# AE-HYU/monte_carlo_localization

Hardware: AMD Instinct MI355X
Metric: MCL updates/sec (particle*beam/s) (higher is better)
Workload: dtype f64; 1 GPU; 4194304 particles/GPU x 1081 beams, Spielberg_map (2000x2000 @ 0.05796), initial cloud N((0.0, 0.0, 0.0),(0.5 m,0.5 m,0.4 rad)) (tracking regime), action (0.05, 0.0, 0.01), stock sensor/motion params, multinomial resampling, Philox seed 42; the timed updates follow 5 warm-up updates (the particle set has resampled to motion-noise width); particles_total=4194304, beams=1081, parallelism=single GPU

## Files before the change

monte_carlo_localization_amd/csrc/mcl_kernels.h:

```cpp
#pragma once
#include "mcl_types.h"
#include <type_traits>
#include "mcl_ray_core.h"
#include "mcl_device_math.h"
#include "mcl_wedge.h"
#include "mcl_motion.h"

namespace mcl {

constexpr int kRedBlocks = 1024;
constexpr int kRedThreads = 256;
__device__ __forceinline__ void final_sums_of(const double *__restrict__ part, int nb, double *__restrict__ scalars, double (*sm)[7]);


__device__ __forceinline__ uint64_t wave_incl_scan_u64(uint64_t v, int lane)
{
#pragma unroll
    for (int o = 1; o < 64; o <<= 1) {
        uint64_t t = (uint64_t)__shfl_up((long long)v, o, 64);
        if (lane >= o) v += t;
    }
    return v;
}

// ... 1204 lines not shown
__global__ __launch_bounds__(1024) void k_tile_compact(int *__restrict__ bbox, int *__restrict__ tilemark, int *__restrict__ tilemap, int ntiles_abs)
{
    __shared__ int ws[16];
    __shared__ int carry_sh;
    const int lane = threadIdx.x & 63, wv = threadIdx.x >> 6;
    if (threadIdx.x == 0) carry_sh = 0;
    __syncthreads();
    for (int t0 = 0; t0 < ntiles_abs; t0 += 1024) {
        const int t = t0 + (int)threadIdx.x;
        const int m = (t < ntiles_abs && tilemark[t] != 0) ? 1 : 0;
        int inc = m;
#pragma unroll
        for (int o = 1; o < 64; o <<= 1) { const int v = __shfl_up(inc, o, 64); if (lane >= o) inc += v; }
        if (lane == 63) ws[wv] = inc;
        __syncthreads();
        int id = carry_sh + inc - m;
        for (int k = 0; k < wv; ++k) id += ws[k];
        if (t < ntiles_abs) { tilemap[t] = m ? id : -1; tilemark[t] = 0; }
        __syncthreads();
        if (threadIdx.x == 1023) carry_sh = id + m;
        __syncthreads();
    }
    const int T = carry_sh;
    for (int t = threadIdx.x; t < ntiles_abs; t += 1024)
        if (tilemap[t] < 0) tilemap[t] = T;
    if (threadIdx.x == 0) { bbox[4] = T; bbox[5] = 1; }
}

#ifndef MCL_SORT_SUB_GATE
#define MCL_SORT_SUB_GATE 32.0
#endif
constexpr double kSortSubGate = MCL_SORT_SUB_GATE;
constexpr int kSortMaxSub = MCL_SORT_MAX_SUB;
struct SortLayout {
    int cs, tb, inner, ss;
    uint32_t ntx;
    int tx0, ty0;
    bool compact;
    bool nocut;
    bool sparse;
    uint64_t ntiles;
    __device__ __forceinline__ int tile_shift() const { return 2 * inner + 2 * ss + tb; }
    __device__ __forceinline__ int cut_shift() const { return sparse ? 2 * ss + tb : tile_shift(); }
    __device__ __forceinline__ uint64_t cut_groups() const { return sparse ? ntiles << (2 * inner) : ntiles; }
    __device__ __forceinline__ bool cuts() const;
};
constexpr int kSwMaxCuts = 65536;
__device__ __forceinline__ bool SortLayout::cuts() const
{
    return compact && !nocut && cut_groups() <= (uint64_t)kSwMaxCuts && (cut_groups() << cut_shift()) <= kSortKeySpace;
}
__device__ __forceinline__ SortLayout sort_layout(const int *__restrict__ bbox, int64_t n)
{
    SortLayout L;
    L.tx0 = bbox[0] >> 5; L.ty0 = bbox[1] >> 5;
    L.ntx = (uint32_t)((bbox[2] >> 5) - L.tx0 + 1);
    const uint32_t nty = (uint32_t)((bbox[3] >> 5) - L.ty0 + 1);
    L.compact = bbox[5] != 0;
    L.ntiles = L.compact ? (uint64_t)bbox[4] + 1u : (uint64_t)L.ntx * nty;
    double cells_est = (double)(bbox[2] - bbox[0] + 1) * (double)(bbox[3] - bbox[1] + 1);
    if (L.compact && (double)bbox[4] * 1024.0 < cells_est) cells_est = (double)bbox[4] * 1024.0;
    int cs = 0, tb = 6;
    L.nocut = bbox[6] < 0;
    L.sparse = cells_est > 0.0 && (double)n < 8.0 * cells_est;
    if (L.sparse) {
        cs = 5;
        const int play = bbox[6];
        while (play > 0 && cs > 1 && (1 << cs) >= play - 2 && (double)n * (double)(1 << (2 * cs - 2)) >= 128.0 * cells_est) --cs;
    }
    while (cs < 5 && ((L.ntiles << (10 - 2 * cs + tb)) > kSortKeySpace)) ++cs;
    while (tb > 0 && ((L.ntiles << (10 - 2 * cs + tb)) > kSortKeySpace)) --tb;
    const int inner = 5 - cs;
    const uint64_t ncell = L.ntiles << (2 * inner);
    while (tb < 8 && (ncell << (tb + 1)) <= kSortKeySpace) ++tb;
    int ss = 0;
    if (cs == 0 && tb == 8) {
        double per_bucket = cells_est > 0.0 ? (double)n / cells_est / 32.0 : 0.0;
        while (ss < kSortMaxSub && (ncell << (tb + 2 * (ss + 1))) <= kSortKeySpace && per_bucket >= kSortSubGate) { ++ss; per_bucket *= 0.25; }
    }
    L.cs = cs; L.tb = tb; L.inner = inner; L.ss = ss;
    return L;
}

__device__ __forceinline__ uint32_t sort_key(const int *__restrict__ bbox, const int *__restrict__ tilemap, int ntx_abs, int cx, int cy, double th,
                                         int64_t n, double fx, double fy)
{
    cx = cx < bbox[0] ? bbox[0] : (cx > bbox[2] ? bbox[2] : cx);
    cy = cy < bbox[1] ? bbox[1] : (cy > bbox[3] ? bbox[3] : cy);
    const SortLayout L = sort_layout(bbox, n);
    const int cs = L.cs, tb = L.tb, inner = L.inner, ss = L.ss;
    uint32_t tile = (uint32_t)((cy >> 5) - L.ty0) * L.ntx + (uint32_t)((cx >> 5) - L.tx0);
    if (L.compact) tile = (uint32_t)tilemap[(cy >> 5) * ntx_abs + (cx >> 5)];
    const uint32_t ix = (uint32_t)(cx & 31) >> cs, iy = (uint32_t)(cy & 31) >> cs;
    uint64_t key = ((((uint64_t)tile << inner) | iy) << inner) | ix;
    if (ss > 0) {
        const uint32_t sx = (fx >= 0.0 && fx < 1.0) ? (uint32_t)(fx * (double)(1 << ss)) : 0u;
        const uint32_t sy = (fy >= 0.0 && fy < 1.0) ? (uint32_t)(fy * (double)(1 << ss)) : 0u;
        key = (((key << ss) | sy) << ss) | sx;
    }
    double f = th * 0.15915494309189533577;
    f -= floor(f);
    uint32_t tq = (f >= 0.0 && f < 1.0) ? (uint32_t)(f * (double)(1u << tb)) : 0u;
    if (tq >> tb) tq = (1u << tb) - 1u;
    key = (key << tb) | tq;
    return key < kSortKeySpace ? (uint32_t)key : kSortKeySpace - 1u;
}

__global__ __launch_bounds__(256) void k_sort_hist(const double4 *__restrict__ pc, const double *__restrict__ th, int64_t n, int Wp, int Hp,
                                                  const int *__restrict__ bbox, uint32_t *__restrict__ hist,
                                                  uint32_t *__restrict__ key_out, uint32_t *__restrict__ rank_out, uint32_t *__restrict__ tile_used,
                                                  const int *__restrict__ tilemap, int ntx_abs)
{
    const int64_t i = (int64_t)blockIdx.x * blockDim.x + threadIdx.x;
    if (i >= n) return;
    const uint32_t xcd = (uint32_t)__builtin_amdgcn_s_getreg((20 << 0) | (0 << 6) | (3 << 11)) & (kSortXcds - 1);
    const double4 c = pc[i];
    const uint32_t key = sort_key(bbox, tilemap, ntx_abs, cell_of(c.z * kSortSub, Wp * kSortSub - 1), cell_of(c.w * kSortSub, Hp * kSortSub - 1), th[i], n,
                                  c.z * kSortSub - floor(c.z * kSortSub), c.w * kSortSub - floor(c.w * kSortSub));
    key_out[i] = key;
    const uint32_t r = __hip_atomic_fetch_add(&hist[(size_t)xcd * kSortKeySpace + key], 1u, __ATOMIC_RELAXED, __HIP_MEMORY_SCOPE_WORKGROUP);
    rank_out[i] = (xcd << 28) | r;
    if (r == 0u) tile_used[key / kHistTile] = 1u;
}

__global__ __launch_bounds__(256) void k_hist_partials(const uint32_t *__restrict__ hist, uint32_t *__restrict__ part, const uint32_t *__restrict__ tile_used)
{
    __shared__ uint32_t ws[4];
    if (!tile_used[blockIdx.x]) {
        if (threadIdx.x == 0) part[blockIdx.x] = 0u;
        return;
    }
    uint32_t s = 0;
    for (int x = 0; x < kSortXcds; ++x) {
        const uint4 *p = reinterpret_cast<const uint4 *>(hist + (size_t)x * kSortKeySpace + (size_t)blockIdx.x * kHistTile) + threadIdx.x * 4;
#pragma unroll
        for (int k = 0; k < 4; ++k) { uint4 v = p[k]; s += v.x + v.y + v.z + v.w; }
    }
#pragma unroll
    for (int o = 32; o > 0; o >>= 1) s += __shfl_xor(s, o, 64);
    if ((threadIdx.x & 63) == 0) ws[threadIdx.x >> 6] = s;
    __syncthreads();
    if (threadIdx.x == 0) part[blockIdx.x] = ws[0] + ws[1] + ws[2] + ws[3];
}

__global__ __launch_bounds__(256) void k_hist_final(uint32_t *__restrict__ hist, const uint32_t *__restrict__ part, const uint32_t *__restrict__ tile_used)
{
    __shared__ uint32_t ws[4], ps[4];
    if (!tile_used[blockIdx.x]) return;
    const int lane = threadIdx.x & 63, w = threadIdx.x >> 6;
    uint32_t pre = 0;
    for (int t = (int)threadIdx.x; t < (int)blockIdx.x; t += 256) pre += part[t];
#pragma unroll
    for (int o = 32; o > 0; o >>= 1) pre += __shfl_xor(pre, o, 64);
    if (lane == 0) ps[w] = pre;
    const size_t b0 = (size_t)blockIdx.x * kHistTile + (size_t)threadIdx.x * 16;
    uint4 v[kSortXcds][4];
    uint32_t s = 0;
#pragma unroll
    for (int x = 0; x < kSortXcds; ++x) {
        const uint4 *p = reinterpret_cast<const uint4 *>(hist + (size_t)x * kSortKeySpace + b0);
#pragma unroll
        for (int k = 0; k < 4; ++k) { v[x][k] = p[k]; s += v[x][k].x + v[x][k].y + v[x][k].z + v[x][k].w; }
    }
    uint32_t inc = s;
#pragma unroll
    for (int o = 1; o < 64; o <<= 1) { uint32_t t = __shfl_up(inc, o, 64); if (lane >= o) inc += t; }
    if (lane == 63) ws[w] = inc;
    __syncthreads();
    uint32_t run = ps[0] + ps[1] + ps[2] + ps[3] + inc - s;
    for (int k = 0; k < w; ++k) run += ws[k];
#pragma unroll
    for (int k = 0; k < 4; ++k) {
#pragma unroll
        for (int x = 0; x < kSortXcds; ++x) { uint32_t c = v[x][k].x; v[x][k].x = run; run += c; }
#pragma unroll
        for (int x = 0; x < kSortXcds; ++x) { uint32_t c = v[x][k].y; v[x][k].y = run; run += c; }
#pragma unroll
        for (int x = 0; x < kSortXcds; ++x) { uint32_t c = v[x][k].z; v[x][k].z = run; run += c; }
#pragma unroll
        for (int x = 0; x < kSortXcds; ++x) { uint32_t c = v[x][k].w; v[x][k].w = run; run += c; }
    }
#pragma unroll
    for (int x = 0; x < kSortXcds; ++x) {
        uint4 *p = reinterpret_cast<uint4 *>(hist + (size_t)x * kSortKeySpace + b0);
#pragma unroll
        for (int k = 0; k < 4; ++k) p[k] = v[x][k];
    }
}

__global__ __launch_bounds__(256) void k_sort_scatter(const double4 *__restrict__ pc, const double *__restrict__ th, int64_t n,
                                                     const uint32_t *__restrict__ key, const uint32_t *__restrict__ rank,
                                                     const uint32_t *__restrict__ start, double4 *__restrict__ pcs,
                                                     double *__restrict__ ths, uint32_t *__restrict__ perm)
{
    const int64_t i = (int64_t)blockIdx.x * blockDim.x + threadIdx.x;
    if (i >= n) return;
    const uint32_t rk = rank[i];
    const uint32_t slot = start[(size_t)(rk >> 28) * kSortKeySpace + key[i]] + (rk & 0x0FFFFFFFu);
    if (slot >= (uint64_t)n) return;
    pcs[slot] = pc[i];
    ths[slot] = th[i];
    perm[slot] = (uint32_t)i;
}

__global__ __launch_bounds__(256) void k_sort_keys(const double4 *__restrict__ pc, const double *__restrict__ th, int64_t n, int Wp, int Hp,
                                                  const int *__restrict__ bbox, uint32_t *__restrict__ key_out, uint32_t *__restrict__ val_out,
                                                  const int *__restrict__ tilemap, int ntx_abs)
{
    const int64_t i = (int64_t)blockIdx.x * blockDim.x + threadIdx.x;
    if (i >= n) return;
    const double4 c = pc[i];
    key_out[i] = sort_key(bbox, tilemap, ntx_abs, cell_of(c.z * kSortSub, Wp * kSortSub - 1), cell_of(c.w * kSortSub, Hp * kSortSub - 1), th[i], n,
                          c.z * kSortSub - floor(c.z * kSortSub), c.w * kSortSub - floor(c.w * kSortSub));
    val_out[i] = (uint32_t)i;
}
__global__ __launch_bounds__(256) void k_sort_gather(const double4 *__restrict__ pc, const double *__restrict__ th, int64_t n,
                                                    const uint32_t *__restrict__ order, double4 *__restrict__ pcs, double *__restrict__ ths,
                                                    uint32_t *__restrict__ perm, const uint32_t *__restrict__ sorted_keys = nullptr,
                                                    const int *__restrict__ bbox = nullptr, uint32_t *__restrict__ cut_start = nullptr,
                                                    uint32_t *__restrict__ cut_end = nullptr)
{
    const int64_t s = (int64_t)blockIdx.x * blockDim.x + threadIdx.x;
    if (s >= n) return;
    const uint32_t i = order[s];
    pcs[s] = pc[i];
    ths[s] = th[i];
    perm[s] = i;
    if (sorted_keys) {
        const SortLayout L = sort_layout(bbox, n);
        if (L.cuts()) {
            const int sh = L.cut_shift();
            const uint32_t g = sorted_keys[s] >> sh;
            const uint32_t gp = s > 0 ? sorted_keys[s - 1] >> sh : 0xFFFFFFFFu;
            if (g != gp && g < (uint32_t)kSwMaxCuts) {
                cut_start[g] = (uint32_t)s + 1u;
                if (s > 0 && gp < (uint32_t)kSwMaxCuts) cut_end[gp] = (uint32_t)s;
            }
            if (s == n - 1 && g < (uint32_t)kSwMaxCuts) cut_end[g] = (uint32_t)n;
        }
    }
}

__global__ __launch_bounds__(256) void k_hist_clear(uint32_t *__restrict__ hist, uint32_t *__restrict__ tile_used)
{
    if (!tile_used[blockIdx.x]) return;
    const uint4 z = make_uint4(0u, 0u, 0u, 0u);
    for (int x = 0; x < kSortXcds; ++x) {
        uint4 *p = reinterpret_cast<uint4 *>(hist + (size_t)x * kSortKeySpace + (size_t)blockIdx.x * kHistTile) + threadIdx.x * 4;
#pragma unroll
        for (int k = 0; k < 4; ++k) p[k] = z;
    }
    __syncthreads();
    if (threadIdx.x == 0) tile_used[blockIdx.x] = 0u;
}

__global__ __launch_bounds__(256) void k_slice_means(const double4 *__restrict__ pcs, int64_t n, int64_t per, double2 *__restrict__ out)
{
    __shared__ double sm[4][3];
    const int64_t p_begin = (int64_t)blockIdx.x * per;
    const int64_t p_end = (p_begin + per < n) ? p_begin + per : n;
    double sx = 0.0, sy = 0.0, cnt = 0.0;
    for (int64_t s = p_begin + threadIdx.x; s < p_end; s += blockDim.x) {
        const double4 c = pcs[s];
        if (c.z == c.z && c.w == c.w && fabs(c.z) < 1e9 && fabs(c.w) < 1e9) { sx += c.z; sy += c.w; cnt += 1.0; }
    }
    sx = wave_sum(sx); sy = wave_sum(sy); cnt = wave_sum(cnt);
    if ((threadIdx.x & 63) == 0) { sm[threadIdx.x >> 6][0] = sx; sm[threadIdx.x >> 6][1] = sy; sm[threadIdx.x >> 6][2] = cnt; }
    __syncthreads();
    if (threadIdx.x == 0) {
        sx = sm[0][0] + sm[1][0] + sm[2][0] + sm[3][0];
        sy = sm[0][1] + sm[1][1] + sm[2][1] + sm[3][1];
        cnt = sm[0][2] + sm[1][2] + sm[2][2] + sm[3][2];
        out[blockIdx.x] = cnt > 0.0 ? make_double2(sx / cnt, sy / cnt) : make_double2(0.0, 0.0);
    }
}

template <bool GRID = false>
__device__ __forceinline__ int first_beam_in_wedge(double th, const float *__restrict__ angle, int B, int m, double a0, double inv_inc)
{
    int lo = 0, hi = B;
    const double x = ((double)m * (6.283185307179586476925286766559 / kWedges) - th - a0) * inv_inc;
    if (x > -4.0 && x < (double)B + 4.0) {
        const int jg = min(max((int)ceil(x), 0), B);
        if (GRID && fabs(x - rint(x)) > 4e-6 * inv_inc + 1e-6) return jg;
        const bool below = jg == 0 || beam_wedge(th, angle[jg - 1]) < m;
        const bool at = jg == B || beam_wedge(th, angle[jg]) >= m;
        if (below && at) return jg;
        const int l = max(jg - 2, 0), h = min(jg + 2, B);
        if ((l == 0 || beam_wedge(th, angle[l - 1]) < m) && (h == B || beam_wedge(th, angle[h]) >= m)) { lo = l; hi = h; }
    }
    while (lo < hi) {
        const int mid = (lo + hi) >> 1;
        if (beam_wedge(th, angle[mid]) >= m) hi = mid; else lo = mid + 1;
    }
    return lo;
}

#ifdef MCL_LEGACY_RAY_KERNELS
}
#include "mcl_rays_legacy.h"
namespace mcl {
#endif

template <bool COUNT>
__global__ __launch_bounds__(256) void k_rays_fix(RayArgs a)
{
    unsigned long long cnt_exact = 0, cnt_probe = 0, cnt_l2 = 0;
    const int split = max(1, (int)gridDim.x / a.fix_segments);
    const int part = blockIdx.x % split;
    for (int seg = blockIdx.x / split; seg < a.fix_segments; seg += gridDim.x / split) {
    unsigned long long n = 0;
    if (threadIdx.x == 0) n = a.slot_space ? a.fix_count[(size_t)seg * 8] : atomicAdd(&a.fix_count[(size_t)seg * 8], 0ull);
    n = __shfl((long long)n, 0, 64);
    {
        __shared__ unsigned long long n_sh;
        if (threadIdx.x == 0) n_sh = n;
        __syncthreads();
        n = n_sh;
        __syncthreads();
    }
    if (n > a.fix_cap) n = 0;
    cnt_l2 += (threadIdx.x == 0 && part == 0) ? n : 0;
    const unsigned long long *list = a.fix_list + (size_t)seg * a.fix_cap;
    for (unsigned long long k = (unsigned long long)part * blockDim.x + threadIdx.x; k < n; k += (unsigned long long)blockDim.x * split) {
        const unsigned long long e = a.slot_space ? list[k] : atomicAdd(const_cast<unsigned long long *>(&list[k]), 0ull);
        const int64_t p = (int64_t)(e >> 16);
        const int j = (int)(e & 0xFFFF);
        const double4 pci = a.slot_space ? a.pcs[p] : a.pc[p];
        const uint8_t *wfield = nullptr;
        if (a.slot_space && a.distw) {
            const double hth = a.ths[p];
            if (hth == hth && fabs(hth) < 1e6) wfield = a.distw + (size_t)(beam_wedge(hth, a.beam_angle[j]) & (kWedges - 1)) * a.distw_stride;
        }
        const double2 cs = a.beam_cs[j];
        const double ux = pci.x * cs.x - pci.y * cs.y, uy = pci.y * cs.x + pci.x * cs.y;
        const RayOrigin o = ray_origin(a, pci.z, pci.w);
        int r = a.P;
        uint32_t amb = o.amb0;
        unsigned np = 0;
        if (o.sane)
            r = trace_fp64<false, COUNT>(a, nullptr, 0, kOriginBase, o.p0x, o.p0y, ux, uy, first_skip(a, o, wfield ? wfield : a.dist, wfield != nullptr),
                                         amb, np, wfield, wfield != nullptr);
        if (takes_literal_march(a, o.sane, amb)) {
            if (a.exact_list) {
                const unsigned long long slot = atomicAdd(a.exact_count, 1ull);
                if (slot < a.exact_cap) { atomicExch(&a.exact_list[slot], e); continue; }
            }
            const int64_t i = a.slot_space ? (int64_t)a.perm[p] : p;
            r = march_exact(a, a.x[i], a.y[i], a.th[i] + (double)a.beam_angle[j]);
            ++cnt_exact;
        }
        atomicAdd(&a.logw[p], (double)a.Lt[(size_t)r * a.bpad + j]);
        if (a.steps || a.steps16) store_step(a, a.slot_space ? (int64_t)a.perm[p] : p, j, r);
        if (COUNT) cnt_probe += np;
    }
    }
    if (a.counters) {
        if (cnt_exact) atomicAdd(&a.counters[0], cnt_exact);
        if (COUNT && cnt_probe) atomicAdd(&a.counters[2], cnt_probe);
        if (cnt_l2) atomicAdd(&a.counters[3], cnt_l2);
    }
}

template <bool COUNT>
__global__ __launch_bounds__(256) void k_rays_exact(RayArgs a)
{
    const int lane = threadIdx.x & 63;
    const unsigned long long wave_id = ((unsigned long long)blockIdx.x * blockDim.x + threadIdx.x) >> 6;
    const unsigned long long nwaves = ((unsigned long long)gridDim.x * blockDim.x) >> 6;
    unsigned long long n = 0;
    if (lane == 0) n = atomicAdd(a.exact_count, 0ull);
    n = (unsigned long long)__shfl((long long)n, 0, 64);
    if (n > a.exact_cap) n = a.exact_cap;
    unsigned long long done = 0;
    for (unsigned long long k = wave_id; k < n; k += nwaves) {
        unsigned long long e = 0;
        if (lane == 0) e = atomicAdd(&a.exact_list[k], 0ull);
        e = (unsigned long long)__shfl((long long)e, 0, 64);
        const int64_t p = (int64_t)(e >> 16);
        const int64_t i = a.slot_space ? (int64_t)a.perm[p] : p;
        const int j = (int)(e & 0xFFFF);
        const double angle = a.th[i] + (double)a.beam_angle[j];
        const double dx = cos(angle) * a.res, dy = sin(angle) * a.res;
        const int r = wave_march_exact_dir(a, a.x[i], a.y[i], dx, dy, lane);
        if (lane == 0) {
            atomicAdd(&a.logw[p], (double)a.Lt[(size_t)r * a.bpad + j]);
            if (a.steps || a.steps16) store_step(a, i, j, r);
            ++done;
        }
    }
    if (a.counters && lane == 0 && done) atomicAdd(&a.counters[0], done);
}

__global__ void k_gather_logw(const double *__restrict__ acc, int64_t n, double *__restrict__ out)
{
    int64_t i = (int64_t)blockIdx.x * blockDim.x + threadIdx.x;
    if (i < n) out[i] = acc[i];
}

__global__ void k_fix_overflow(const unsigned long long *__restrict__ counts, int nseg, unsigned long long cap, unsigned long long *over)
{
    __shared__ unsigned int s;
    if (threadIdx.x == 0) s = 0;
    __syncthreads();
    unsigned int c = 0;
    for (int k = threadIdx.x; k < nseg; k += blockDim.x)
        c += atomicAdd(const_cast<unsigned long long *>(&counts[(size_t)k * 8]), 0ull) > cap ? 1u : 0u;
    if (c) atomicAdd(&s, c);
    __syncthreads();
    if (threadIdx.x == 0) *over = s;
}

constexpr int kFarTile = 2048;
__global__ __launch_bounds__(256) void k_far_count(const uint32_t *__restrict__ flags32, int64_t n, const unsigned long long *__restrict__ far_count,
                                                  uint32_t *__restrict__ cnt)
{
    if (*far_count < kFarWindowedMin) return;
    __shared__ uint32_t ws[4];
    const int64_t base = (int64_t)blockIdx.x * kFarTile + (int64_t)threadIdx.x * 8;
    uint32_t c = 0;
#pragma unroll
    for (int k = 0; k < 8; ++k) c += (base + k < n && flags32[base + k] != 0u) ? 1u : 0u;
#pragma unroll
    for (int o = 32; o > 0; o >>= 1) c += __shfl_xor(c, o, 64);
    if ((threadIdx.x & 63) == 0) ws[threadIdx.x >> 6] = c;
    __syncthreads();
    if (threadIdx.x == 0) cnt[blockIdx.x] = ws[0] + ws[1] + ws[2] + ws[3];
}
__global__ __launch_bounds__(1024) void k_far_spine(uint32_t *__restrict__ cnt, int nb, const unsigned long long *__restrict__ far_count)
{
    if (*far_count < kFarWindowedMin) return;
    __shared__ uint32_t ws[16];
    __shared__ uint32_t carry_sh;
    const int lane = threadIdx.x & 63, wv = threadIdx.x >> 6;
    if (threadIdx.x == 0) carry_sh = 0u;
    __syncthreads();
    for (int b0 = 0; b0 < nb; b0 += 1024) {
        const int i = b0 + (int)threadIdx.x;
        const uint32_t v = i < nb ? cnt[i] : 0u;
        uint32_t inc = v;
#pragma unroll
        for (int o = 1; o < 64; o <<= 1) { const uint32_t t = __shfl_up(inc, o, 64); if (lane >= o) inc += t; }
        if (lane == 63) ws[wv] = inc;
        __syncthreads();
        uint32_t at = carry_sh + inc - v;
        for (int k = 0; k < wv; ++k) at += ws[k];
        if (i < nb) cnt[i] = at;
        __syncthreads();
        if (threadIdx.x == 1023) carry_sh = at + v;
        __syncthreads();
    }
}
__global__ __launch_bounds__(256) void k_far_scatter(const uint32_t *__restrict__ flags32, int64_t n, const unsigned long long *__restrict__ far_count,
                                                    const uint32_t *__restrict__ cnt_excl, uint32_t *__restrict__ out)
{
    if (*far_count < kFarWindowedMin) return;
    __shared__ uint32_t ws[4];
    const int lane = threadIdx.x & 63, wv = threadIdx.x >> 6;
    const int64_t base = (int64_t)blockIdx.x * kFarTile + (int64_t)threadIdx.x * 8;
    uint32_t m = 0;
#pragma unroll
    for (int k = 0; k < 8; ++k) m |= ((base + k < n && flags32[base + k] != 0u) ? 1u : 0u) << k;
    const uint32_t c = (uint32_t)__popc(m);
    uint32_t inc = c;
#pragma unroll
    for (int o = 1; o < 64; o <<= 1) { const uint32_t t = __shfl_up(inc, o, 64); if (lane >= o) inc += t; }
    if (lane == 63) ws[wv] = inc;
    __syncthreads();
    uint32_t at = cnt_excl[blockIdx.x] + inc - c;
    for (int k = 0; k < wv; ++k) at += ws[k];
#pragma unroll
    for (int k = 0; k < 8; ++k)
        if ((m >> k) & 1u) out[at++] = (uint32_t)(base + k);
}

template <bool COUNT>
__global__ __launch_bounds__(kRayThreads, 8) void k_rays_far(RayArgs a)
{
    const int lane = threadIdx.x & 63;
    const int wave = __builtin_amdgcn_readfirstlane(threadIdx.x >> 6);
    const int64_t p_end = a.n;
    unsigned long long cnt_exact = 0, cnt_off = 0, cnt_probe = 0;
    const uint32_t *flags32 = reinterpret_cast<const uint32_t *>(a.far_flags);
    if (a.far_windowed && a.far_count && *a.far_count >= kFarWindowedMin) return;
    const int64_t n_list = a.far_list ? (int64_t)min((unsigned long long)a.n, *a.far_count) : 0;
    const int64_t wave_global = (int64_t)wave * gridDim.x + blockIdx.x, waves_total = (int64_t)kRayWaves * gridDim.x;
    for (int64_t i0 = a.far_list ? wave_global : wave_global * 64; i0 < (a.far_list ? n_list : p_end); i0 += a.far_list ? waves_total : waves_total * 64) {
      uint32_t myfl;
      unsigned long long todo;
      int64_t listed = 0;
      if (a.far_list) {
          listed = (int64_t)a.far_list[i0];
          myfl = flags32[listed];
          todo = 1ull;
      } else {
          myfl = (i0 + lane < p_end) ? flags32[i0 + lane] : 0u;
          todo = __ballot(myfl != 0u);
      }
      while (todo) {
        const int src = __ffsll((long long)todo) - 1;
        todo &= todo - 1;
        const int64_t p = a.far_list ? listed : i0 + src;
        const int64_t i = a.slot_space ? (int64_t)a.perm[p] : p;
        const uint32_t fl = a.far_list ? myfl : (uint32_t)__shfl((int)myfl, src, 64);
        if (lane == 0) ++cnt_off;
        const double4 pci = a.slot_space ? a.pcs[p] : a.pc[p];
        const double cth = pci.x, sth = pci.y, gpx = pci.z, gpy = pci.w;
        const bool sane = (gpx > -200000.0) && (gpx < 200000.0) && (gpy > -200000.0) && (gpy < 200000.0);
        const double p0x = (gpx + 1.0 + 262144.0) + kMagic, p0y = (gpy + 1.0 + 262144.0) + kMagic;
        const int base = kOriginBase;
        uint32_t amb0 = 0;
        int cx0 = 0, cy0 = 0;
        bool in0 = false;
        if (sane) {
            uint32_t lox = (uint32_t)__double2loint(p0x), loy = (uint32_t)__double2loint(p0y);
            cx0 = (__double2hiint(p0x) & 0xFFFFF) - base; cy0 = (__double2hiint(p0y) & 0xFFFFF) - base;
            amb0 = lox < loy ? lox : loy;
            in0 = (unsigned)cx0 < (unsigned)a.Wp && (unsigned)cy0 < (unsigned)a.Hp;
        }
        short4 qr;
        if (a.qr) qr = a.qr[i];
        else { const double t = a.th[i]; qr = quadrant_ranges_of(t, t == t && fabs(t) < 1e6, a.beam_angle, a.B); }
        double acc = 0.0;
        for (int q = 0; q < 4; ++q) {
            if (((fl >> (8 * q)) & 0xFFu) == 0) continue;
            const uint8_t *field = a.distq[q];
            const int d0 = in0 ? field[(size_t)cy0 * a.Wps + cx0] : 0;
            const int s0 = d0 > 1 ? d0 : 1;
            int ja, jb, ja2;
            quad_ranges(qr, q, a.B, ja, jb, ja2);
            for (int seg = 0; seg < 2; ++seg)
            for (int j0 = seg ? ja2 : ja, je = seg ? a.B : jb; j0 < je; j0 += 64) {
                int j = j0 + lane;
                if (j < je) {
                    int r = a.P;
                    unsigned np = 0;
                    uint32_t amb = amb0;
                    if (sane) {
                        double2 cs = a.beam_cs[j];
                        double ux = cth * cs.x - sth * cs.y;
                        double uy = sth * cs.x + cth * cs.y;
                        r = trace_fp64<false, COUNT>(a, nullptr, 0, base, p0x, p0y, ux, uy, s0, amb, np, field);
                    }
                    if (takes_literal_march(a, sane, amb)) {
                        r = march_exact(a, a.x[i], a.y[i], a.th[i] + (double)a.beam_angle[j]);
                        ++cnt_exact;
                    }
                    acc += (double)a.Lt[(size_t)r * a.bpad + j];
                    if (a.steps || a.steps16) store_step(a, i, j, r);
                    if (COUNT) cnt_probe += np;
                }
            }
        }
        acc = wave_sum(acc);
        if (lane == 0) atomicAdd(&a.logw[p], acc);
      }
    }
    if (a.counters) {
        cnt_exact = wave_sum_u64(cnt_exact);
        cnt_off = wave_sum_u64(cnt_off);
        cnt_probe = wave_sum_u64(cnt_probe);
        if (lane == 0) {
            if (cnt_exact) atomicAdd(&a.counters[0], cnt_exact);
            if (cnt_off) atomicAdd(&a.counters[1], cnt_off);
            if (COUNT && cnt_probe) atomicAdd(&a.counters[2], cnt_probe);
        }
    }
}

__global__ void k_product_weights(const uint8_t *__restrict__ steps, const uint16_t *__restrict__ steps16, const int32_t *__restrict__ obs_idx, int64_t n, int B,
                                  const double *__restrict__ table , int tw, double inv_squash,
                                  double *__restrict__ w_out)
{
    int64_t i = (int64_t)blockIdx.x * blockDim.x + threadIdx.x;
    if (i >= n) return;
    double w = 1.0;
    for (int j = 0; j < B; ++j) w *= table[(size_t)(steps16 ? (int)steps16[(size_t)i * B + j] : (int)steps[(size_t)i * B + j]) * tw + obs_idx[j]];
    w_out[i] = pow(w, inv_squash);
}

__global__ __launch_bounds__(kRedThreads) void k_reduce_max(const double *__restrict__ v, int64_t n, double *__restrict__ part)
{
    __shared__ double sm[kRedThreads / 64];
    double m = -INFINITY;
    for (int64_t i = (int64_t)blockIdx.x * kRedThreads + threadIdx.x; i < n; i += (int64_t)gridDim.x * kRedThreads)
        m = fmax(m, v[i]);
    m = wave_max(m);
    if ((threadIdx.x & 63) == 0) sm[threadIdx.x >> 6] = m;
    __syncthreads();
    if (threadIdx.x == 0) {
        for (int k = 1; k < kRedThreads / 64; ++k) m = fmax(m, sm[k]);
        part[blockIdx.x] = m;
    }
}
__global__ __launch_bounds__(kRedThreads) void k_final_max(const double *__restrict__ part, int nb, double *__restrict__ out,
                                                           double *__restrict__ out2)
{
    __shared__ double sm[kRedThreads / 64];
    double m = -INFINITY;
    for (int i = threadIdx.x; i < nb; i += kRedThreads) m = fmax(m, part[i]);
    m = wave_max(m);
    if ((threadIdx.x & 63) == 0) sm[threadIdx.x >> 6] = m;
    __syncthreads();
    if (threadIdx.x == 0) {
        for (int k = 1; k < kRedThreads / 64; ++k) m = fmax(m, sm[k]);
        out[0] = m;
        if (out2) out2[0] = m;
    }
}

__global__ void k_copy_double(const double *__restrict__ src, double *__restrict__ dst) { dst[0] = src[0]; }
__global__ void k_set_double(double *__restrict__ dst, double v) { dst[0] = v; }
__global__ void k_spin_ms(double ms)
{
    const unsigned long long t0 = __builtin_amdgcn_s_memrealtime();
    const unsigned long long ticks = (unsigned long long)((ms < 2000.0 ? ms : 2000.0) * 1e5);
    while (__builtin_amdgcn_s_memrealtime() - t0 < ticks) __builtin_amdgcn_s_sleep(64);
}

__global__ void k_group_max(GroupMaxArgs a)
{
    double m = -INFINITY;
    for (int i = 0; i < a.n; ++i) m = fmax(m, a.src[i][0]);
    a.out[0] = m;
}

__global__ void k_stage_pack(const unsigned long long *__restrict__ res, double *__restrict__ vec, int n_shards, int self, int listed,
                             unsigned long long list_cap)
// ... 250 lines not shown
```

Baseline: 897.6 billion particle*beam/s.

## Flatten fix-list work across segments with block prefix scan in slot-space path

In slot-space mode, each block now reads the counts of up to 1024 fix segments, builds an exclusive prefix sum in shared memory, and spreads the combined entries over all threads of the grid. Each thread finds its segment by binary search over the prefix array. Before this, blocks were split statically across segments, which left threads idle when segment counts were uneven. The launch bounds also gain a minimum of 8 blocks per CU, which may limit registers in the trace code.

```diff
diff --git a/monte_carlo_localization_amd/csrc/mcl_kernels.h b/monte_carlo_localization_amd/csrc/mcl_kernels.h
--- a/monte_carlo_localization_amd/csrc/mcl_kernels.h
+++ b/monte_carlo_localization_amd/csrc/mcl_kernels.h
@@ -1530,15 +1530,44 @@
 namespace mcl {
 #endif
 
+constexpr int kFixBatch = 1024;
 template <bool COUNT>
-__global__ __launch_bounds__(256) void k_rays_fix(RayArgs a)
+__global__ __launch_bounds__(256, 8) void k_rays_fix(RayArgs a)
 {
     unsigned long long cnt_exact = 0, cnt_probe = 0, cnt_l2 = 0;
+    static_assert(kFixBatch == 4 * 256, "four counts per thread of the 256 the kernel is launched with");
+    __shared__ unsigned long long pre_sh[kFixBatch + 1], wtot_sh[4];
     const int split = max(1, (int)gridDim.x / a.fix_segments);
     const int part = blockIdx.x % split;
-    for (int seg = blockIdx.x / split; seg < a.fix_segments; seg += gridDim.x / split) {
-    unsigned long long n = 0;
-    if (threadIdx.x == 0) n = a.slot_space ? a.fix_count[(size_t)seg * 8] : atomicAdd(&a.fix_count[(size_t)seg * 8], 0ull);
+    const unsigned long long t0 = (unsigned long long)blockIdx.x * blockDim.x + threadIdx.x, nt = (unsigned long long)gridDim.x * blockDim.x;
+    for (int seg = a.slot_space ? 0 : blockIdx.x / split; seg < a.fix_segments; seg += a.slot_space ? kFixBatch : gridDim.x / split) {
+    unsigned long long n = 0, k0, kstep;
+    const int ns = min(kFixBatch, a.fix_segments - seg);
+    if (a.slot_space) {
+        const int lane = threadIdx.x & 63, wv = threadIdx.x >> 6;
+        if (seg) __syncthreads();
+        unsigned long long c[4], sum = 0;
+#pragma unroll
+        for (int q = 0; q < 4; ++q) {
+            const int k = (int)threadIdx.x * 4 + q;
+            unsigned long long v = k < ns ? a.fix_count[(size_t)(seg + k) * 8] : 0ull;
+            if (v > a.fix_cap) v = 0;
+            c[q] = v; sum += v;
+        }
+        const unsigned long long inc = wave_incl_scan_u64(sum, lane);
+        if (lane == 63) wtot_sh[wv] = inc;
+        __syncthreads();
+        unsigned long long ex = inc - sum;
+        for (int k = 0; k < wv; ++k) ex += wtot_sh[k];
+#pragma unroll
+        for (int q = 0; q < 4; ++q) { pre_sh[threadIdx.x * 4 + q] = ex; ex += c[q]; }
+        if (threadIdx.x == 255) pre_sh[kFixBatch] = ex;
+        __syncthreads();
+        n = pre_sh[kFixBatch];
+        cnt_l2 += t0 == 0 ? n : 0;
+        k0 = t0; kstep = nt;
+    } else {
+    if (threadIdx.x == 0) n = atomicAdd(&a.fix_count[(size_t)seg * 8], 0ull);
     n = __shfl((long long)n, 0, 64);
     {
         __shared__ unsigned long long n_sh;
@@ -1549,9 +1578,18 @@
     }
     if (n > a.fix_cap) n = 0;
     cnt_l2 += (threadIdx.x == 0 && part == 0) ? n : 0;
+    k0 = (unsigned long long)part * blockDim.x + threadIdx.x; kstep = (unsigned long long)blockDim.x * split;
+    }
     const unsigned long long *list = a.fix_list + (size_t)seg * a.fix_cap;
-    for (unsigned long long k = (unsigned long long)part * blockDim.x + threadIdx.x; k < n; k += (unsigned long long)blockDim.x * split) {
-        const unsigned long long e = a.slot_space ? list[k] : atomicAdd(const_cast<unsigned long long *>(&list[k]), 0ull);
+    for (unsigned long long k = k0; k < n; k += kstep) {
+        unsigned long long e;
+        if (a.slot_space) {
+            int lo = 0, hi = ns;
+            while (hi - lo > 1) { const int mid = (lo + hi) >> 1; if (pre_sh[mid] <= k) lo = mid; else hi = mid; }
+            e = list[(size_t)lo * a.fix_cap + (k - pre_sh[lo])];
+        } else {
+            e = atomicAdd(const_cast<unsigned long long *>(&list[k]), 0ull);
+        }
         const int64_t p = (int64_t)(e >> 16);
         const int j = (int)(e & 0xFFFF);
         const double4 pci = a.slot_space ? a.pcs[p] : a.pc[p];
```

Result: no change. 899.1 billion particle*beam/s, median of 5 (+0.2%).
